# sloisel/LinearAlgebraMPI.jl

Hardware: AMD Instinct MI355X
Metric: SpMV GFLOP/s (2*nnz/t), 2-D 5-pt Poisson, fp64 (higher is better)
Workload: dtype f64

## Files before the change

include/hpcla_rocm.h:

```cpp
#ifndef HPCLA_ROCM_H
#define HPCLA_ROCM_H

#include <stdint.h>

#ifdef __cplusplus
extern "C" {
#endif

#define HPCLA_VERSION 100

#define HPCLA_OK 0
#define HPCLA_ERR_INVALID -1
#define HPCLA_ERR_HIP -2
#define HPCLA_ERR_RCCL -3
#define HPCLA_ERR_NO_DEVICE -4
#define HPCLA_ERR_UNSUPPORTED -5
#define HPCLA_ERR_ALLOC -6

#define HPCLA_LAYOUT_ROW 0
#define HPCLA_LAYOUT_COL 1

typedef struct hpcla_comm hpcla_comm_t;
typedef struct hpcla_halo_plan hpcla_halo_plan_t;

int hpcla_version(void);
const char *hpcla_last_error(void);
int hpcla_device_count(int *count);
int hpcla_set_device(int device);
int hpcla_device_info(int device, int *num_cus, char *arch_name_host, int arch_name_len);

int hpcla_spmv_csr_f64_i32(const int32_t *rowptr, const int32_t *colval, const double *nzval,
                           const double *x, double *y, int64_t nrows, int64_t nnz, int index_base,
                           void *stream);
int hpcla_spmv_csr_f64_i64(const int64_t *rowptr, const int64_t *colval, const double *nzval,
                           const double *x, double *y, int64_t nrows, int64_t nnz, int index_base,
                           void *stream);

int hpcla_spmv_split_f64_i32(const int32_t *rowptr, const int32_t *colval_split,
                             const double *nzval, const double *x_own, const double *x_ghost,
                             int64_t n_own, double *y, int64_t nrows, int64_t nnz, int index_base,
                             const int32_t *block_list, int64_t n_blocks, void *stream);
int hpcla_spmv_split_f64_i64(const int64_t *rowptr, const int64_t *colval_split,
                             const double *nzval, const double *x_own, const double *x_ghost,
                             int64_t n_own, double *y, int64_t nrows, int64_t nnz, int index_base,
                             const int32_t *block_list, int64_t n_blocks, void *stream);
int hpcla_spmv_rows_per_block(void);
int64_t hpcla_spmv_longrows_work_bytes(int64_t n_long);
int hpcla_spmv_longrows_f64_i32(const int32_t *rowptr, const int32_t *colval_split, const double *nzval,
                                const double *x_own, const double *x_ghost, int64_t n_own, double *y,
                                int64_t nrows, int64_t nnz, int index_base, const int64_t *long_rows,
                                int64_t n_long, int64_t long_min, double *work, void *stream);
int hpcla_spmv_longrows_f64_i64(const int64_t *rowptr, const int64_t *colval_split, const double *nzval,
                                const double *x_own, const double *x_ghost, int64_t n_own, double *y,
                                int64_t nrows, int64_t nnz, int index_base, const int64_t *long_rows,
                                int64_t n_long, int64_t long_min, double *work, void *stream);
int hpcla_spmm_rows_per_block(void);
int hpcla_spmm_block_order_hint(const void *rowptr, int group);
int hpcla_spmm_tune_block_order_f64_i32(const int32_t *rowptr, const int32_t *colval_split, const double *nzval,
                                        const double *B_own, int64_t ldb_own, const double *B_ghost, int64_t ldb_ghost,
                                        int64_t n_own, double *C, int64_t ldc, int64_t nrows, int64_t nnz, int k,
                                        int index_base, const int32_t *block_list, int64_t n_blocks, void *stream,
                                        int *chosen_group);
int hpcla_spmm_tune_block_order_f64_i64(const int64_t *rowptr, const int64_t *colval_split, const double *nzval,
                                        const double *B_own, int64_t ldb_own, const double *B_ghost, int64_t ldb_ghost,
                                        int64_t n_own, double *C, int64_t ldc, int64_t nrows, int64_t nnz, int k,
                                        int index_base, const int32_t *block_list, int64_t n_blocks, void *stream,
                                        int *chosen_group);

int hpcla_spmv_block_order_hint(const void *rowptr, int group);

int hpcla_spmv_tune_block_order_f64_i32(const int32_t *rowptr, const int32_t *colval_split, const double *nzval,
                                        const double *x_own, const double *x_ghost, int64_t n_own, double *y_scratch,
                                        int64_t nrows, int64_t nnz, int index_base, void *stream, int *chosen_group);
int hpcla_spmv_tune_block_order_f64_i64(const int64_t *rowptr, const int64_t *colval_split, const double *nzval,
                                        const double *x_own, const double *x_ghost, int64_t n_own, double *y_scratch,
                                        int64_t nrows, int64_t nnz, int index_base, void *stream, int *chosen_group);

int hpcla_remap_i32(const int32_t *in, const int32_t *map, int32_t *out, int64_t n, int index_base,
                    void *stream);
int hpcla_remap_i64(const int64_t *in, const int64_t *map, int64_t *out, int64_t n, int index_base,
                    void *stream);
int hpcla_remap_i64_to_i32(const int64_t *in, const int32_t *map, int32_t *out, int64_t n, int index_base,
                           void *stream);
int hpcla_narrow_i64_to_i32(const int64_t *in, int32_t *out, int64_t n, uint32_t *overflow_dev, void *stream);
int hpcla_classify_blocks_i32(const int32_t *rowptr, const int32_t *colval_split, int64_t nrows,
                              int index_base, int64_t n_own, int rows_per_block, int32_t *flags,
                              void *stream);
int hpcla_classify_blocks_i64(const int64_t *rowptr, const int64_t *colval_split, int64_t nrows,
                              int index_base, int64_t n_own, int rows_per_block, int32_t *flags,
                              void *stream);

int64_t hpcla_colspace_work_bytes(int64_t window);
int hpcla_digest_i32(const int32_t *a, int64_t n, uint64_t *out_host , void *stream);
int hpcla_digest_i64(const int64_t *a, int64_t n, uint64_t *out_host , void *stream);
int hpcla_compress_columns_i32(const int64_t *colidx_global, int64_t nnz, int64_t col_lo, int64_t window,
                               int32_t *colval_out, int index_base, int64_t *col_indices_out,
                               int64_t *ncols_compressed_host, void *work, void *stream);
int hpcla_compress_columns_i64(const int64_t *colidx_global, int64_t nnz, int64_t col_lo, int64_t window,
                               int64_t *colval_out, int index_base, int64_t *col_indices_out,
                               int64_t *ncols_compressed_host, void *work, void *stream);
int64_t hpcla_poisson2d_nnz(int64_t nx, int64_t ny, int64_t row_start, int64_t row_end);
int hpcla_gen_poisson2d(int64_t nx, int64_t ny, int64_t row_start, int64_t row_end, int64_t *rowptr_out,
                        int64_t *colidx_out, double *vals_out, void *stream);
int64_t hpcla_poisson3d_nnz(int64_t nx, int64_t ny, int64_t nz, int64_t row_start, int64_t row_end);
int hpcla_gen_poisson3d(int64_t nx, int64_t ny, int64_t nz, int64_t row_start, int64_t row_end,
                        int64_t *rowptr_out, int64_t *colidx_out, double *vals_out, void *stream);

int64_t hpcla_submatrix_work_bytes(int64_t nsel, int64_t width);
int64_t hpcla_submatrix_scan_chunk(void);
int hpcla_submatrix_structure_i32(const int32_t *rowptr, const int32_t *colval, int64_t nrows, int64_t nnz, int64_t r0,
                                  int64_t r1, int64_t j0, int64_t j1, int index_base, const int64_t *col_indices_src,
                                  int64_t col_shift, int64_t *src_start_out, int32_t *rowptr_out, int64_t *col_indices_out,
                                  int64_t *nnz_out_host, int64_t *ncols_out_host, void *work, void *stream);
int hpcla_submatrix_structure_i64(const int64_t *rowptr, const int64_t *colval, int64_t nrows, int64_t nnz, int64_t r0,
                                  int64_t r1, int64_t j0, int64_t j1, int index_base, const int64_t *col_indices_src,
                                  int64_t col_shift, int64_t *src_start_out, int64_t *rowptr_out, int64_t *col_indices_out,
                                  int64_t *nnz_out_host, int64_t *ncols_out_host, void *work, void *stream);
int hpcla_submatrix_fill_i32(int elem_bytes, const int32_t *colval, const void *nzval, int64_t nnz_src,
                             const int64_t *src_start, const int32_t *rowptr_out, int64_t nsel, int64_t nnz_out, int64_t j0,
                             int64_t j1, int index_base, const void *work, int32_t *colval_out, void *nzval_out, void *stream);
int hpcla_submatrix_fill_i64(int elem_bytes, const int64_t *colval, const void *nzval, int64_t nnz_src,
                             const int64_t *src_start, const int64_t *rowptr_out, int64_t nsel, int64_t nnz_out, int64_t j0,
                             int64_t j1, int index_base, const void *work, int64_t *colval_out, void *nzval_out, void *stream);
int hpcla_submatrix_values_i32(int elem_bytes, const void *nzval, int64_t nnz_src, const int64_t *src_start,
                               const int32_t *rowptr_out, int64_t nsel, int64_t nnz_out, int index_base, void *nzval_out,
                               void *stream);
int hpcla_submatrix_values_i64(int elem_bytes, const void *nzval, int64_t nnz_src, const int64_t *src_start,
                               const int64_t *rowptr_out, int64_t nsel, int64_t nnz_out, int index_base, void *nzval_out,
                               void *stream);
// ... 708 lines not shown
```

linearalgebrampi.jl_amd/_capi.py:

```python
from __future__ import annotations

import ctypes
import os

_HERE = os.path.dirname(os.path.abspath(__file__))
LIB_PATH = os.path.join(_HERE, "libhpcla_rocm.so")

OK = 0
LAYOUT_ROW = 0
LAYOUT_COL = 1
UNIQUE_ID_BYTES = 128
WINDOW_DESC_BYTES = 128
WINDOW_TABLE_ROWS = 4
COMM_NO_RCCL = 1
HALO_SINGLE_BUFFER = 1
BLOCK_PATTERNS_WEAK_HASH = 1


class HPCLAError(RuntimeError):
    def __init__(self, fn: str, status: int, text: str):
        super().__init__(f"{fn} failed with status {status}: {text}")
        self.status = status


_lib = None

_i32 = ctypes.c_int
_i64 = ctypes.c_int64
_u64 = ctypes.c_uint64
_f64 = ctypes.c_double
_f32 = ctypes.c_float
_vp = ctypes.c_void_p

_SIGNATURES = {
    "hpcla_version": [],
    "hpcla_last_error": [],
    "hpcla_device_count": [_vp],
    "hpcla_set_device": [_i32],
    "hpcla_device_info": [_i32, _vp, _vp, _i32],
    "hpcla_spmv_csr_f64_i32": [_vp, _vp, _vp, _vp, _vp, _i64, _i64, _i32, _vp],
    "hpcla_spmv_csr_f64_i64": [_vp, _vp, _vp, _vp, _vp, _i64, _i64, _i32, _vp],
    "hpcla_spmv_split_f64_i32": [_vp, _vp, _vp, _vp, _vp, _i64, _vp, _i64, _i64, _i32, _vp, _i64, _vp],
    "hpcla_spmv_split_f64_i64": [_vp, _vp, _vp, _vp, _vp, _i64, _vp, _i64, _i64, _i32, _vp, _i64, _vp],
    "hpcla_spmv_rows_per_block": [],
    "hpcla_spmv_longrows_work_bytes": [_i64],
    "hpcla_spmv_longrows_f64_i32": [_vp, _vp, _vp, _vp, _vp, _i64, _vp, _i64, _i64, _i32, _vp, _i64, _i64, _vp, _vp],
    "hpcla_spmv_longrows_f64_i64": [_vp, _vp, _vp, _vp, _vp, _i64, _vp, _i64, _i64, _i32, _vp, _i64, _i64, _vp, _vp],
    "hpcla_spmv_block_order_hint": [_vp, _i32],
    "hpcla_spmv_tune_block_order_f64_i32": [_vp, _vp, _vp, _vp, _vp, _i64, _vp, _i64, _i64, _i32, _vp, _vp],
    "hpcla_spmv_tune_block_order_f64_i64": [_vp, _vp, _vp, _vp, _vp, _i64, _vp, _i64, _i64, _i32, _vp, _vp],
    "hpcla_spmv_tune_block_order_cols16_f64_i32": [_vp, _vp, _vp, _vp, _vp, _i64, _i64, _i32, _i64, _i64, _vp, _vp],
    "hpcla_cols16_padded_len": [_i64],
    "hpcla_cols16_encode_i32": [_vp, _vp, _i64, _i64, _i64, _i32, _vp, _i64, _vp, _vp, _vp],
    "hpcla_spmv_cols16_f64_i32": [_vp, _vp, _vp, _vp, _vp, _i64, _i64, _i32, _vp, _i64, _vp],
    "hpcla_block_patterns_create_i32": [_vp, _vp, _vp, _i64, _i64, _i32, _vp, _i64, _i64, _i32, _vp],
    "hpcla_block_patterns_destroy": [_vp],
    "hpcla_block_patterns_info": [_vp, _vp, _vp, _vp, _vp],
    "hpcla_spmv_patterns_f64_i32": [_vp, _vp, _vp, _vp, _vp, _vp, _i64, _i64, _i32, _vp, _i64, _vp],
    "hpcla_spmv_tune_block_order_patterns_f64_i32": [_vp, _vp, _vp, _vp, _vp, _vp, _i64, _i64, _i32, _i64, _i64, _vp, _vp],
    "hpcla_spmm_rows_per_block": [],
    "hpcla_spmm_runs_desc_bytes": [_i64],
    "hpcla_spmm_runs_build_i32": [_vp, _vp, _i64, _i64, _i32, _i64, _vp, _vp, _vp],
    "hpcla_spmm_runs_build_i64": [_vp, _vp, _i64, _i64, _i32, _i64, _vp, _vp, _vp],
    "hpcla_spmm_banded_blocks_i32": [_vp, _vp, _i64, _i64, _i32, _i64, _i32, _vp, _vp],
    "hpcla_spmm_banded_blocks_i64": [_vp, _vp, _i64, _i64, _i32, _i64, _i32, _vp, _vp],
    "hpcla_spmm_runs_k16_f64_i32": [_vp, _vp, _vp, _vp, _vp, _i64, _vp, _i64, _i64, _i32, _vp, _vp, _i64, _vp],
    "hpcla_spmm_runs_k16_f64_i64": [_vp, _vp, _vp, _vp, _vp, _i64, _vp, _i64, _i64, _i32, _vp, _vp, _i64, _vp],
    "hpcla_spmm_runs_colmajor_k16_f64_i32": [_vp, _vp, _vp, _vp, _i64, _vp, _i64, _i64, _vp, _i64, _i64, _i64, _i32, _vp, _vp, _i64, _vp],
    "hpcla_spmm_runs_colmajor_k16_f64_i64": [_vp, _vp, _vp, _vp, _i64, _vp, _i64, _i64, _vp, _i64, _i64, _i64, _i32, _vp, _vp, _i64, _vp],
    "hpcla_spmm_runs_colmajor_tune_block_order_f64_i32": [_vp, _vp, _vp, _vp, _i64, _vp, _i64, _i64, _vp, _i64, _i64, _i64, _i32, _vp, _vp, _i64, _vp, _vp],
    "hpcla_spmm_runs_colmajor_tune_block_order_f64_i64": [_vp, _vp, _vp, _vp, _i64, _vp, _i64, _i64, _vp, _i64, _i64, _i64, _i32, _vp, _vp, _i64, _vp, _vp],
    "hpcla_spmm_block_order_hint": [_vp, _i32],
    "hpcla_spmm_tune_block_order_f64_i32": [_vp, _vp, _vp, _vp, _i64, _vp, _i64, _i64, _vp, _i64, _i64, _i64, _i32, _i32,
                                            _vp, _i64, _vp, _vp],
    "hpcla_spmm_tune_block_order_f64_i64": [_vp, _vp, _vp, _vp, _i64, _vp, _i64, _i64, _vp, _i64, _i64, _i64, _i32, _i32,
                                            _vp, _i64, _vp, _vp],
    "hpcla_remap_i32": [_vp, _vp, _vp, _i64, _i32, _vp],
    "hpcla_remap_i64": [_vp, _vp, _vp, _i64, _i32, _vp],
    "hpcla_remap_i64_to_i32": [_vp, _vp, _vp, _i64, _i32, _vp],
    "hpcla_narrow_i64_to_i32": [_vp, _vp, _i64, _vp, _vp],
    "hpcla_classify_blocks_i32": [_vp, _vp, _i64, _i32, _i64, _i32, _vp, _vp],
    "hpcla_classify_blocks_i64": [_vp, _vp, _i64, _i32, _i64, _i32, _vp, _vp],
    "hpcla_spmm_csr_f64_i32": [_vp, _vp, _vp, _vp, _i64, _i32, _vp, _i64, _i32, _i64, _i64, _i32, _i32, _vp],
    "hpcla_spmm_csr_f64_i64": [_vp, _vp, _vp, _vp, _i64, _i32, _vp, _i64, _i32, _i64, _i64, _i32, _i32, _vp],
    "hpcla_spmm_split_f64_i32": [_vp, _vp, _vp, _vp, _i64, _vp, _i64, _i64, _vp, _i64, _i64, _i64, _i32, _i32, _vp, _i64, _vp],
    "hpcla_spmm_split_f64_i64": [_vp, _vp, _vp, _vp, _i64, _vp, _i64, _i64, _vp, _i64, _i64, _i64, _i32, _i32, _vp, _i64, _vp],
    "hpcla_spmm_split_ccol_f64_i32": [_vp, _vp, _vp, _vp, _i64, _vp, _i64, _i64, _vp, _i64, _i64, _i64, _i32, _i32, _vp, _i64, _vp],
    "hpcla_spmm_split_ccol_f64_i64": [_vp, _vp, _vp, _vp, _i64, _vp, _i64, _i64, _vp, _i64, _i64, _i64, _i32, _i32, _vp, _i64, _vp],
    "hpcla_spmm_split_colmajor_f64_i32": [_vp, _vp, _vp, _vp, _i64, _vp, _i64, _i64, _vp, _i64, _i64, _i64, _i32, _i32, _vp, _i64, _vp],
    "hpcla_spmm_split_colmajor_f64_i64": [_vp, _vp, _vp, _vp, _i64, _vp, _i64, _i64, _vp, _i64, _i64, _i64, _i32, _i32, _vp, _i64, _vp],
    "hpcla_halo_begin_strided_f64": [_vp, _vp, _i64, _i64, _vp, _vp],
    "hpcla_spmm_panel_f64_i32": [_vp, _vp, _vp, _vp, _i64, _vp, _i64, _i64, _vp, _i64, _i64, _i64, _i32, _i32, _i32, _vp],
    "hpcla_spmm_panel_f64_i64": [_vp, _vp, _vp, _vp, _i64, _vp, _i64, _i64, _vp, _i64, _i64, _i64, _i32, _i32, _i32, _vp],
    "hpcla_transpose_f64": [_vp, _i64, _i32, _vp, _i64, _i32, _i64, _i64, _vp],
    "hpcla_gather_f64_i32": [_vp, _vp, _vp, _vp, _i64, _i32, _vp],
    "hpcla_gather_f64_i64": [_vp, _vp, _vp, _vp, _i64, _i32, _vp],
    "hpcla_comm_get_unique_id": [_vp],
    "hpcla_comm_init_rank": [_vp, _vp, _i32, _i32],
    "hpcla_comm_init_rank_ex": [_vp, _vp, _i32, _i32, _i32],
    "hpcla_comm_window_export": [_vp, _vp],
    "hpcla_comm_window_attach": [_vp, _vp],
# ... 259 lines not shown
    "hpcla_spmv_dot_work_bytes": _i64,
    "hpcla_colspace_work_bytes": _i64,
    "hpcla_submatrix_work_bytes": _i64,
    "hpcla_submatrix_scan_chunk": _i64,
    "hpcla_poisson2d_nnz": _i64,
    "hpcla_poisson3d_nnz": _i64,
    "hpcla_spgemm_bin_cap": _i64,
    "hpcla_gemv_t_work_bytes": _i64,
    "hpcla_gram_work_bytes": _i64,
    "hpcla_spmm_t_struct_work_bytes": _i64,
    "hpcla_spmm_runs_desc_bytes": _i64,
    "hpcla_spmv_longrows_work_bytes": _i64,
    "hpcla_cols16_padded_len": _i64,
    "hpcla_pcg_work_bytes": _i64,
    "hpcla_fsai_work_bytes": _i64,
    "hpcla_ilu_work_bytes": _i64,
    "hpcla_amg_work_bytes": _i64,
    "hpcla_amg_round_blocks": _i64,
    "hpcla_bicgstab_work_bytes": _i64,
    "hpcla_lsqr_work_bytes": _i64,
    "hpcla_minres_work_bytes": _i64,
    "hpcla_gmres_work_bytes": _i64,
    "hpcla_gmres_small_offset": _i64,
    "hpcla_eigsh_small_offset": _i64,
    "hpcla_svds_small_offset": _i64,
    "hpcla_lobpcg_chunk_rows": _i64,
    "hpcla_lobpcg_work_bytes": _i64,
    "hpcla_lobpcg_gen_work_bytes": _i64,
    "hpcla_qr_work_bytes": _i64,
}

EXPORTED_SYMBOLS = tuple(_SIGNATURES)


def load() -> ctypes.CDLL:
    global _lib
    if _lib is not None:
        return _lib
    if not os.path.exists(LIB_PATH):
        raise ImportError(
            f"{LIB_PATH} not found: build it with `python -c 'import __graft_entry__ as g; g.build()'` "
            "or `make -C linearalgebrampi.jl_amd/csrc` (hipcc --offload-arch=gfx950). "
            "There is no CPU fallback.")
    try:
        import torch
    except Exception:
        pass
    lib = ctypes.CDLL(LIB_PATH, mode=ctypes.RTLD_GLOBAL)
    for name, argtypes in _SIGNATURES.items():
        fn = getattr(lib, name)
        fn.argtypes = argtypes
        fn.restype = _RESTYPES.get(name, ctypes.c_int)
    _lib = lib
    return lib


def last_error() -> str:
    s = load().hpcla_last_error()
    return s.decode("utf-8", "replace") if s else ""


def check(fn_name: str, status: int) -> None:
    if status != OK:
        raise HPCLAError(fn_name, status, last_error())


def call(fn_name: str, *args) -> None:
    check(fn_name, getattr(load(), fn_name)(*args))
```

linearalgebrampi.jl_amd/csrc/spmv.hip:

```cpp
#include <stdlib.h>
#include <string.h>

#include <atomic>
#include <mutex>
#include <type_traits>
#include <unordered_map>

#include "common.h"
#include "halo_wait.h"
#include "patterns.h"

namespace hpcla {

constexpr int RPB = 256;
static_assert(RPB == PAT_RPB, "the pattern table is built for this kernel's row blocks");
constexpr int CHUNK = RPB * 8;
constexpr int UNROLL = CHUNK / RPB;

template <typename T, int N>
using vec = T __attribute__((ext_vector_type(N)));

struct Cols16 {};
struct Pat16 {};
template <typename P>
struct IndexPolicy {
    using row_t = P;
    using col_t = P;
    static constexpr int VEC = 4;
    static constexpr bool PATTERNS = false;
    static __device__ __forceinline__ int64_t decode(col_t c, int base, int64_t ) { return (int64_t)(P)(c - (P)base); }
    static __device__ __forceinline__ col_t fill(int base) { return (P)base; }
};
template <>
struct IndexPolicy<Cols16> {
    using row_t = int32_t;
    using col_t = int16_t;
    static constexpr int VEC = 8;
    static constexpr bool PATTERNS = false;
    static __device__ __forceinline__ int64_t decode(col_t d, int , int64_t r0) { return r0 + (int)d; }
    static __device__ __forceinline__ col_t fill(int ) { return 0; }
};
template <>
struct IndexPolicy<Pat16> : IndexPolicy<Cols16> {
    static constexpr bool PATTERNS = true;
};

template <bool SPLIT>
__device__ __forceinline__ double gather_x(const double *__restrict__ x_own,
                                           const double *__restrict__ x_ghost, int64_t n_own,
                                           int64_t col)
{
    if (SPLIT) {
        const double *p = col < n_own ? x_own + col : x_ghost + (col - n_own);
        return *p;
    }
    return x_own[col];
}

struct BlockSel {
    const int32_t *list;
    int64_t base;
    const int32_t *first_list;
    int64_t first_base;
    int64_t n_first;
    int64_t n_run;
    int32_t group_log2;
    int32_t nt_y;
};

constexpr int NUM_XCD_LOG2 = 3;
__device__ __forceinline__ int64_t xcd_group_index(int64_t b, int64_t n, int group_log2)
{
    const int64_t span = (int64_t)1 << (NUM_XCD_LOG2 + group_log2);
    if (b >= n - (n & (span - 1))) return b;
    const int64_t xcd = b & ((1 << NUM_XCD_LOG2) - 1), q = b >> NUM_XCD_LOG2;
    return ((((q >> group_log2) << NUM_XCD_LOG2) + xcd) << group_log2) + (q & (((int64_t)1 << group_log2) - 1));
}

template <bool WAIT>
__device__ __forceinline__ int64_t select_block(const BlockSel &bs, bool &wait, int lead)
{
    const int64_t b = (int64_t)blockIdx.x - lead;
    wait = false;
    if (WAIT) {
        if (b < bs.n_first) {
            if (bs.first_list) return (int64_t)bs.first_list[b];
            return bs.first_base + (bs.group_log2 > 0 ? xcd_group_index(b, bs.n_run, bs.group_log2) : b);
        }
        wait = true;
        return bs.list ? (int64_t)bs.list[b - bs.n_first] : bs.base + (b - bs.n_first);
    }
    if (bs.list) return (int64_t)bs.list[b];
    return bs.base + (bs.group_log2 > 0 ? xcd_group_index(b, bs.n_run, bs.group_log2) : b);
}

__device__ __forceinline__ void block_dot_epilogue(double *s_scratch, double *__restrict__ dot_partial,
                                                   int64_t blk, double v)
{
#pragma unroll
    for (int off = 32; off > 0; off >>= 1) v += __shfl_down(v, off, 64);
    const int lane = threadIdx.x & 63, w = threadIdx.x >> 6;
    if (lane == 0) s_scratch[w] = v;
    __syncthreads();
    if (threadIdx.x == 0) dot_partial[blk] = ((s_scratch[0] + s_scratch[1]) + s_scratch[2]) + s_scratch[3];
}

constexpr int RG_CHW = 464;
constexpr int RG_UR = 8;

template <typename I, bool SPLIT, bool WAIT, bool LONGR = false>
__global__ __launch_bounds__(RPB) void spmv_rowgather_kernel(
    const typename IndexPolicy<I>::row_t *__restrict__ rowptr, const typename IndexPolicy<I>::col_t *__restrict__ colval,
    const double *__restrict__ nzval, const double *__restrict__ x_own, const double *x_ghost, int64_t n_own,
    double *__restrict__ y, int64_t nrows, int64_t nnz, int base,
    BlockSel bs, double *__restrict__ dot_partial, HaloWait hw, PushArgs push, int64_t long_min = 0, PatArgs pat = PatArgs{nullptr, nullptr})
{
    using IP = IndexPolicy<I>;
    using R = typename IP::row_t;
    using C = typename IP::col_t;
    constexpr int V = IP::VEC;
    constexpr int NV = (RG_CHW / V + 63) / 64;
    static_assert(!LONGR || !WAIT, "the long-row form is a plain launch");
    static_assert(V * sizeof(C) == 16 || sizeof(C) == 8, "one 16-byte column load per staged vector (Int64: two)");
    static_assert(RG_CHW % V == 0 && RG_CHW >= 64 * 7 + V - 1, "a pass holds a 7-entry stencil's wave behind any aligned start");
    __shared__ __attribute__((aligned(16))) C s_col_all[(RPB / 64) * RG_CHW];
    __shared__ __attribute__((aligned(16))) double s_val_all[(RPB / 64) * RG_CHW];
    __shared__ double s_red[RPB / 64];

    if constexpr (WAIT) {
        if ((int)blockIdx.x < push.n_blocks) {
            halo_push_block<R, RPB>(push, (int)blockIdx.x);
            return;
        }
    }
    const int tid = threadIdx.x;
    bool wait_ghosts;
    const int64_t blk = select_block<WAIT>(bs, wait_ghosts, WAIT ? push.n_blocks : 0);
    uint32_t waited = 0;
    if (WAIT && wait_ghosts) {
        waited = halo_wait_block(hw, hw.first_wait_reader + (uint32_t)(blockIdx.x - push.n_blocks - bs.n_first));
        x_ghost = hw.ghost0 + (int64_t)(waited & ~HALO_WAIT_TIMED_OUT) * hw.buf_stride;
    }
    const int64_t r0 = blk * RPB;
    const int nr = (int)((nrows - r0) < RPB ? (nrows - r0) : RPB);
    if (WAIT && (waited & HALO_WAIT_TIMED_OUT)) {
        if ((int)threadIdx.x < nr) y[r0 + threadIdx.x] = halo_poison();
// ... 86 lines not shown
            {
                R blo = rlo, bhi = rhi;
                if constexpr (IP::PATTERNS)
                    if (!streamed) {
                        blo = roff + (R)((uint32_t)rlo & 0xffffu);
                        bhi = roff + (R)((uint32_t)rlo >> 16);
                    }
                const int64_t lo64 = lane < nrw ? (int64_t)blo - base - pa - c : 0;
                const int64_t hi64 = lane < nrw ? (int64_t)bhi - base - pa - c : 0;
                const int lo = lo64 < 0 ? 0 : (lo64 > n ? n : (int)lo64);
                const int hi = hi64 < 0 ? 0 : (hi64 > n ? n : (int)hi64);
                const uint64_t whole = __ballot(lane < nrw && lo == 0 && hi == n && !(LONGR && is_long));
                if (whole) {
#pragma unroll 4
                    for (int e = lane; e < n; e += 64)
                        s_val[e] = s_val[e] * gather_x<SPLIT>(x_own, x_ghost, n_own, IP::decode(s_col[e], base, r0));
                    __builtin_amdgcn_fence(__ATOMIC_RELEASE, "wavefront");
                    __builtin_amdgcn_wave_barrier();
                    if (lane == __ffsll((unsigned long long)whole) - 1) {
                        int j = 0;
#pragma unroll 1
                        for (; j + 4 <= n; j += 4) {
                            const double p0 = s_val[j], p1 = s_val[j + 1], p2 = s_val[j + 2], p3 = s_val[j + 3];
                            acc += p0; acc += p1; acc += p2; acc += p3;
                        }
#pragma unroll 1
                        for (; j < n; ++j) acc += s_val[j];
                    }
                    __builtin_amdgcn_fence(__ATOMIC_ACQUIRE, "wavefront");
                    __builtin_amdgcn_wave_barrier();
                    continue;
                }
                int j = lo;
                int e = hi;
                if (LONGR && is_long) e = j;
                for (; j < e; j += RG_UR) {
                    int64_t cc[RG_UR];
                    double vv[RG_UR], xx[RG_UR];
#pragma unroll
                    for (int u = 0; u < RG_UR; ++u) {
                        cc[u] = 0; vv[u] = 0.0;
                        if (j + u < e) { cc[u] = IP::decode(s_col[j + u], base, r0); vv[u] = s_val[j + u]; }
                    }
#pragma unroll
                    for (int u = 0; u < RG_UR; ++u) { xx[u] = 0.0; if (j + u < e) xx[u] = gather_x<SPLIT>(x_own, x_ghost, n_own, cc[u]); }
#pragma unroll
                    for (int u = 0; u < RG_UR; ++u) if (j + u < e) acc += vv[u] * xx[u];
                }
            }
            __builtin_amdgcn_fence(__ATOMIC_ACQUIRE, "wavefront");
            __builtin_amdgcn_wave_barrier();
        }
        if (lane < nrw && !(LONGR && is_long)) {
            if (bs.nt_y) __builtin_nontemporal_store(acc, y + rw + lane);
            else y[rw + lane] = acc;
        } else if (LONGR && lane < nrw) {
            y[rw + lane] = __builtin_nan("");
        }
    }
    if (dot_partial) block_dot_epilogue(s_red, dot_partial, blk, lane < nrw ? acc * x_row : 0.0);
}

constexpr int LR_CHUNKS = 1024;
constexpr int64_t LR_MIN_CHUNK = 4096;

template <typename I, bool SPLIT>
__global__ __launch_bounds__(256) void spmv_longrow_partial_kernel(
    const I *__restrict__ rowptr, const I *__restrict__ colval, const double *__restrict__ nzval,
    const double *__restrict__ x_own, const double *x_ghost, int64_t n_own, int base,
    const int64_t *__restrict__ long_rows, double *__restrict__ partial)
{
    __shared__ double s_w[4];
    const int64_t r = long_rows[blockIdx.y];
    const int64_t p0 = (int64_t)rowptr[r] - base, p1 = (int64_t)rowptr[r + 1] - base, len = p1 - p0;
    int64_t chunk = (len + LR_CHUNKS - 1) / LR_CHUNKS;
    if (chunk < LR_MIN_CHUNK) chunk = LR_MIN_CHUNK;
    const int64_t s = p0 + (int64_t)blockIdx.x * chunk;
    const int64_t e = s + chunk < p1 ? s + chunk : p1;
    double a0 = 0.0, a1 = 0.0, a2 = 0.0, a3 = 0.0;
    int64_t i = s + threadIdx.x;
    for (; i + 768 < e; i += 1024) {
        const int64_t c0 = (int64_t)(I)(colval[i] - (I)base), c1 = (int64_t)(I)(colval[i + 256] - (I)base),
                      c2 = (int64_t)(I)(colval[i + 512] - (I)base), c3 = (int64_t)(I)(colval[i + 768] - (I)base);
        const double v0 = nzval[i], v1 = nzval[i + 256], v2 = nzval[i + 512], v3 = nzval[i + 768];
        a0 += v0 * gather_x<SPLIT>(x_own, x_ghost, n_own, c0);
        a1 += v1 * gather_x<SPLIT>(x_own, x_ghost, n_own, c1);
        a2 += v2 * gather_x<SPLIT>(x_own, x_ghost, n_own, c2);
        a3 += v3 * gather_x<SPLIT>(x_own, x_ghost, n_own, c3);
    }
    for (; i < e; i += 256) a0 += nzval[i] * gather_x<SPLIT>(x_own, x_ghost, n_own, (int64_t)(I)(colval[i] - (I)base));
    double v = (a0 + a1) + (a2 + a3);
#pragma unroll
    for (int off = 32; off > 0; off >>= 1) v += __shfl_down(v, off, 64);
    if ((threadIdx.x & 63) == 0) s_w[threadIdx.x >> 6] = v;
    __syncthreads();
    if (threadIdx.x == 0) partial[(int64_t)blockIdx.y * LR_CHUNKS + blockIdx.x] = ((s_w[0] + s_w[1]) + s_w[2]) + s_w[3];
}

__global__ __launch_bounds__(256) void spmv_longrow_final_kernel(const int64_t *__restrict__ long_rows,
                                                                 const double *__restrict__ partial, double *__restrict__ y)
{
    __shared__ double s_w[4];
    static_assert(LR_CHUNKS == 1024, "four pieces per thread");
    const double *p = partial + (int64_t)blockIdx.x * LR_CHUNKS + threadIdx.x * 4;
    double v = ((p[0] + p[1]) + p[2]) + p[3];
#pragma unroll
    for (int off = 32; off > 0; off >>= 1) v += __shfl_down(v, off, 64);
// ... 114 lines not shown
    if (threadIdx.x == 0) flags[blockIdx.x] = any ? 1 : 0;
}

template <typename I>
__global__ __launch_bounds__(256) void gather_kernel(const double *__restrict__ x,
                                                     const I *__restrict__ src,
                                                     const I *__restrict__ dst,
                                                     double *__restrict__ out, int64_t n, int base)
{
    int64_t i = (int64_t)blockIdx.x * blockDim.x + threadIdx.x;
    const int64_t stride = (int64_t)gridDim.x * blockDim.x;
    for (; i < n; i += stride) {
        const int64_t d = dst ? (int64_t)dst[i] - base : i;
        out[d] = x[(int64_t)src[i] - base];
    }
}

static inline uint32_t stream_grid(int64_t n, int threads)
{
    int64_t g = (n + threads - 1) / threads;
    if (g < 1) g = 1;
    if (g > 256 * 16) g = 256 * 16;
    return (uint32_t)g;
}

static std::mutex g_order_mu;
static std::unordered_map<const void *, int> g_order;
static std::atomic<int> g_order_count{0};

static int block_order_of(const void *rowptr)
{
    static const int forced = [] {
        const char *e = getenv("HPCLA_SPMV_XCD_GROUP");
        int g = e ? atoi(e) : 0, l = 0;
        while (g > 1) { g >>= 1; ++l; }
        return l > 10 ? 10 : l;
    }();
    if (forced) return forced;
    if (g_order_count.load(std::memory_order_relaxed) == 0) return 0;
    std::lock_guard<std::mutex> lock(g_order_mu);
    auto it = g_order.find(rowptr);
    return it == g_order.end() ? 0 : it->second;
}

static int spmv_nt_y(bool )
{
    static const int on = [] {
        const char *e = getenv("HPCLA_SPMV_NT_Y");
        return e ? (atoi(e) ? 1 : 0) : 1;
    }();
    return on;
}

template <typename I>
static int spmv_launch(const typename IndexPolicy<I>::row_t *rowptr, const typename IndexPolicy<I>::col_t *colval,
                       const double *nzval, const double *x_own,
                       const double *x_ghost, int64_t n_own, bool split, double *y, int64_t nrows,
                       int64_t nnz, int index_base, const int32_t *block_list, int64_t n_blocks,
                       void *stream, double *dot_partial = nullptr, int64_t block_base = -1, const PatArgs *pat = nullptr)
{
    if (nrows < 0 || nnz < 0) return set_error(HPCLA_ERR_INVALID, "spmv: negative size");
    if (index_base != 0 && index_base != 1)
        return set_error(HPCLA_ERR_INVALID, "spmv: index_base must be 0 or 1");
    if (nrows == 0) return HPCLA_OK;
    if (!rowptr || !y) return set_error(HPCLA_ERR_INVALID, "spmv: null rowptr/y");
    if (nnz > 0 && (!colval || !nzval || !x_own))
        return set_error(HPCLA_ERR_INVALID, "spmv: null colval/nzval/x with nnz > 0");
    const int64_t all_blocks = (nrows + RPB - 1) / RPB;
    int64_t launch_blocks = all_blocks;
    if (block_list) {
        if (n_blocks < 0 || n_blocks > all_blocks)
            return set_error(HPCLA_ERR_INVALID, "spmv: n_blocks out of range");
        launch_blocks = n_blocks;
        block_base = 0;
    } else if (block_base >= 0) {
        if (n_blocks < 0 || block_base + n_blocks > all_blocks)
            return set_error(HPCLA_ERR_INVALID, "spmv: block range out of bounds");
        launch_blocks = n_blocks;
    } else {
        block_base = 0;
    }
    if (launch_blocks == 0) return HPCLA_OK;
    if (launch_blocks > 0x7fffffffLL) return set_error(HPCLA_ERR_INVALID, "spmv: too many blocks");
    dim3 grid((uint32_t)launch_blocks), block(RPB);
    hipStream_t s = as_stream(stream);
    if (split && !x_ghost) split = false;
    using IP = IndexPolicy<I>;
    const bool aligned = (reinterpret_cast<uintptr_t>(colval) % (IP::VEC * sizeof(typename IP::col_t)) == 0) &&
                         (reinterpret_cast<uintptr_t>(nzval) % 32 == 0);
    const BlockSel bs{block_list, block_base, nullptr, 0, 0, launch_blocks, block_list ? 0 : block_order_of(rowptr),
                      spmv_nt_y(dot_partial != nullptr)};
    HaloWait nowait;
    memset(&nowait, 0, sizeof(nowait));
    PushArgs nopush;
    memset(&nopush, 0, sizeof(nopush));
    if constexpr (std::is_same<I, Cols16>::value) {
        if (!aligned) return set_error(HPCLA_ERR_INVALID, "spmv: 16-bit columns need a 16-byte aligned copy and 32-byte aligned nzval");
        if (pat)
            spmv_rowgather_kernel<Pat16, false, false><<<grid, block, 0, s>>>(
                rowptr, colval, nzval, x_own, nullptr, 0, y, nrows, nnz, index_base, bs, dot_partial, nowait, nopush, 0, *pat);
        else
            spmv_rowgather_kernel<Cols16, false, false><<<grid, block, 0, s>>>(
                rowptr, colval, nzval, x_own, nullptr, 0, y, nrows, nnz, index_base, bs, dot_partial, nowait, nopush);
    } else if (aligned) {
        if (split)
            spmv_rowgather_kernel<I, true, false><<<grid, block, 0, s>>>(
                rowptr, colval, nzval, x_own, x_ghost, n_own, y, nrows, nnz, index_base, bs, dot_partial, nowait, nopush);
        else
            spmv_rowgather_kernel<I, false, false><<<grid, block, 0, s>>>(
                rowptr, colval, nzval, x_own, nullptr, 0, y, nrows, nnz, index_base, bs, dot_partial, nowait, nopush);
    } else {
        if (split)
            spmv_rowblock_kernel<I, true, false><<<grid, block, 0, s>>>(
                rowptr, colval, nzval, x_own, x_ghost, n_own, y, nrows, index_base, bs, dot_partial, nowait, nopush);
        else
            spmv_rowblock_kernel<I, false, false><<<grid, block, 0, s>>>(
                rowptr, colval, nzval, x_own, nullptr, 0, y, nrows, index_base, bs, dot_partial, nowait, nopush);
    }
    HPCLA_CHECK_LAUNCH();
    return HPCLA_OK;
}

template <typename I>
static int spmv_launch_fused(const I *rowptr, const I *colval, const double *nzval, const double *x_own,
                             const double *x_ghost, int64_t n_own, double *y, int64_t nrows, int64_t nnz,
                             int index_base, const int32_t *interior_list, int64_t interior_base,
                             int64_t n_interior, const int32_t *boundary_list, int64_t n_boundary,
                             const HaloWait &hw, const PushArgs &pa, void *stream, double *dot_partial)
{
    if (nrows < 0 || nnz < 0) return set_error(HPCLA_ERR_INVALID, "spmv: negative size");
    if (index_base != 0 && index_base != 1)
        return set_error(HPCLA_ERR_INVALID, "spmv: index_base must be 0 or 1");
    if (nrows > 0 && (!rowptr || !y)) return set_error(HPCLA_ERR_INVALID, "spmv: null rowptr/y");
    if (nnz > 0 && (!colval || !nzval || !x_own))
        return set_error(HPCLA_ERR_INVALID, "spmv: null colval/nzval/x with nnz > 0");
    const int64_t all_blocks = (nrows + RPB - 1) / RPB;
    if (n_interior < 0 || n_boundary < 0 || n_interior + n_boundary > all_blocks)
        return set_error(HPCLA_ERR_INVALID, "spmv: block counts out of range");
    if (n_boundary > 0 && !boundary_list) return set_error(HPCLA_ERR_INVALID, "spmv: null boundary list");
    if (n_boundary > 0 && !x_ghost) return set_error(HPCLA_ERR_INVALID, "spmv: boundary blocks without a ghost segment");
    if (!interior_list && n_interior > 0 && (interior_base < 0 || interior_base + n_interior > all_blocks))
        return set_error(HPCLA_ERR_INVALID, "spmv: interior run out of bounds");
    const int64_t launch_blocks = pa.n_blocks + n_interior + n_boundary;
    if (launch_blocks == 0) return HPCLA_OK;
    if (launch_blocks > 0x7fffffffLL) return set_error(HPCLA_ERR_INVALID, "spmv: too many blocks");
    dim3 grid((uint32_t)launch_blocks), block(RPB);
    hipStream_t s = as_stream(stream);
    const bool aligned = (reinterpret_cast<uintptr_t>(colval) % (4 * sizeof(I)) == 0) &&
                         (reinterpret_cast<uintptr_t>(nzval) % 32 == 0);
    const BlockSel bs{boundary_list, 0, interior_list, interior_base, n_interior, n_interior,
// ... 59 lines not shown
    for (int64_t j = p0 + threadIdx.x; j < p1; j += 256) {
        const int64_t c = (int64_t)colval[j] - base;
        const int64_t d = c - r0;
        if (c < 0 || c >= n_own || d < -32768 || d > 32767) bad = 1;
        dcol[j] = (int16_t)d;
    }
    if (__syncthreads_or(bad) && threadIdx.x == 0) atomicOr(flags, 1);
}

int64_t cols16_padded_len(int64_t nnz) { return ((nnz + 7) / 8) * 8 + 8; }

int encode_cols16_i32(const int32_t *rowptr, const int32_t *colval, int64_t nrows, int index_base, int64_t n_own,
                      const int32_t *block_list, int64_t n_blocks, int16_t *dcol, int *flag_dev, void *stream)
{
    if (n_blocks <= 0) return HPCLA_OK;
    encode_cols_kernel<<<(uint32_t)n_blocks, 256, 0, as_stream(stream)>>>(rowptr, colval, nrows, index_base, n_own, block_list,
                                                                         dcol, flag_dev);
    HPCLA_CHECK_LAUNCH();
    return HPCLA_OK;
}

int patterns_args(const hpcla_block_patterns *p, int64_t nrows, int64_t nnz, int index_base, PatArgs *out);

bool cols16_usable(const int16_t *cols16, const double *nzval)
{
    return cols16 && reinterpret_cast<uintptr_t>(cols16) % 16 == 0 && reinterpret_cast<uintptr_t>(nzval) % 32 == 0;
}

int spmv_cols16_i32(const int32_t *rowptr, const int16_t *cols16, const double *nzval, const double *x, double *y,
                    int64_t nrows, int64_t nnz, int index_base, const int32_t *bl, int64_t nb, void *stream,
                    double *dot_partial, int64_t block_base, const hpcla_block_patterns *patterns)
{
    PatArgs pa;
    if (patterns)
        if (const int rc = patterns_args(patterns, nrows, nnz, index_base, &pa)) return rc;
    return spmv_launch<Cols16>(rowptr, cols16, nzval, x, nullptr, 0, false, y, nrows, nnz, index_base, bl, nb, stream,
                               dot_partial, block_base, patterns ? &pa : nullptr);
}

}

using namespace hpcla;

HPCLA_API int hpcla_spmv_rows_per_block(void) { return RPB; }

static void set_block_order(const void *rowptr, int group_log2)
{
    std::lock_guard<std::mutex> lock(g_order_mu);
    if (group_log2 <= 0) g_order.erase(rowptr);
    else g_order[rowptr] = group_log2;
    g_order_count.store((int)g_order.size(), std::memory_order_relaxed);
}

template <typename I>
static int tune_block_order(const typename IndexPolicy<I>::row_t *rowptr, const typename IndexPolicy<I>::col_t *colval_split,
                            const double *nzval, const double *x_own,
                            const double *x_ghost, int64_t n_own, double *y_scratch, int64_t nrows, int64_t nnz,
                            int index_base, void *stream, int *chosen_group, int64_t run_base = -1, int64_t run_blocks = 0,
                            const PatArgs *pat = nullptr)
{
    if (chosen_group) *chosen_group = 1;
    if (nrows < 0 || nnz < 0 || !rowptr) return set_error(HPCLA_ERR_INVALID, "spmv_tune_block_order: bad arguments");
    set_block_order(rowptr, 0);
    const int64_t n_blocks = (nrows + RPB - 1) / RPB;
    if (n_blocks < 4096 || nnz == 0) return HPCLA_OK;
    if (run_base >= 0 && (run_blocks <= 0 || run_base + run_blocks > n_blocks))
        return run_blocks == 0 ? HPCLA_OK : set_error(HPCLA_ERR_INVALID, "spmv_tune_block_order: block run out of bounds");
    if (!y_scratch) return set_error(HPCLA_ERR_INVALID, "spmv_tune_block_order: null scratch vector");
    constexpr int NC = 4, ROUNDS = 4, REPS = 4;
    const int cand[NC] = {0, 3, 5, 6};
    float ms[NC][ROUNDS];
    hipEvent_t e0, e1;
    HPCLA_CHECK_HIP(hipEventCreate(&e0));
    HPCLA_CHECK_HIP(hipEventCreate(&e1));
    hipStream_t s = as_stream(stream);
    int rc = HPCLA_OK;
    for (int r = 0; r < ROUNDS && rc == HPCLA_OK; ++r)
        for (int c = 0; c < NC && rc == HPCLA_OK; ++c) {
            set_block_order(rowptr, cand[c]);
            if (hipEventRecord(e0, s) != hipSuccess) { rc = set_error(HPCLA_ERR_HIP, "spmv_tune_block_order: event"); break; }
            for (int i = 0; i < REPS && rc == HPCLA_OK; ++i)
                rc = spmv_launch<I>(rowptr, colval_split, nzval, x_own, x_ghost, n_own, true, y_scratch, nrows, nnz,
                                    index_base, nullptr, run_base >= 0 ? run_blocks : 0, stream, nullptr, run_base, pat);
            if (rc != HPCLA_OK) break;
            if (hipEventRecord(e1, s) != hipSuccess || hipEventSynchronize(e1) != hipSuccess ||
                hipEventElapsedTime(&ms[c][r], e0, e1) != hipSuccess)
                rc = set_error(HPCLA_ERR_HIP, "spmv_tune_block_order: timing");
        }
    (void)hipEventDestroy(e0);
    (void)hipEventDestroy(e1);
    set_block_order(rowptr, 0);
    if (rc != HPCLA_OK) return rc;
    float best_t[NC];
    for (int c = 0; c < NC; ++c) {
        float a = ms[c][1], b = ms[c][2], d = ms[c][3];
        best_t[c] = a > b ? (b > d ? b : (a > d ? d : a)) : (a > d ? a : (b > d ? d : b));
    }
    int best = 0;
    for (int c = 1; c < NC; ++c)
        if (best_t[c] < best_t[best]) best = c;
    if (best != 0 && best_t[best] > 0.99f * best_t[0]) best = 0;
    set_block_order(rowptr, cand[best]);
    if (chosen_group) *chosen_group = 1 << cand[best];
    return HPCLA_OK;
}

HPCLA_API int hpcla_spmv_tune_block_order_f64_i32(const int32_t *rowptr, const int32_t *colval_split, const double *nzval,
                                                  const double *x_own, const double *x_ghost, int64_t n_own,
                                                  double *y_scratch, int64_t nrows, int64_t nnz, int index_base,
                                                  void *stream, int *chosen_group)
{
    return tune_block_order<int32_t>(rowptr, colval_split, nzval, x_own, x_ghost, n_own, y_scratch, nrows, nnz, index_base,
                                     stream, chosen_group);
}

HPCLA_API int hpcla_spmv_tune_block_order_f64_i64(const int64_t *rowptr, const int64_t *colval_split, const double *nzval,
                                                  const double *x_own, const double *x_ghost, int64_t n_own,
                                                  double *y_scratch, int64_t nrows, int64_t nnz, int index_base,
                                                  void *stream, int *chosen_group)
{
    return tune_block_order<int64_t>(rowptr, colval_split, nzval, x_own, x_ghost, n_own, y_scratch, nrows, nnz, index_base,
                                     stream, chosen_group);
}

HPCLA_API int hpcla_spmv_tune_block_order_cols16_f64_i32(const int32_t *rowptr, const int16_t *cols16, const double *nzval,
                                                         const double *x_own, double *y_scratch, int64_t nrows, int64_t nnz,
                                                         int index_base, int64_t block_base, int64_t n_blocks, void *stream,
                                                         int *chosen_group)
{
    if (!cols16_usable(cols16, nzval))
        return set_error(HPCLA_ERR_INVALID, "spmv_tune_block_order_cols16: null or misaligned column copy / nzval");
    return tune_block_order<Cols16>(rowptr, cols16, nzval, x_own, nullptr, 0, y_scratch, nrows, nnz, index_base, stream,
                                    chosen_group, block_base, n_blocks);
}

HPCLA_API int hpcla_spmv_tune_block_order_patterns_f64_i32(const int32_t *rowptr, const int16_t *cols16,
                                                           const hpcla_block_patterns_t *patterns, const double *nzval,
                                                           const double *x_own, double *y_scratch, int64_t nrows, int64_t nnz,
                                                           int index_base, int64_t block_base, int64_t n_blocks, void *stream,
                                                           int *chosen_group)
{
    if (!cols16_usable(cols16, nzval))
        return set_error(HPCLA_ERR_INVALID, "spmv_tune_block_order_patterns: null or misaligned column copy / nzval");
    PatArgs pa;
    if (patterns)
        if (const int rc = patterns_args(patterns, nrows, nnz, index_base, &pa)) return rc;
    return tune_block_order<Cols16>(rowptr, cols16, nzval, x_own, nullptr, 0, y_scratch, nrows, nnz, index_base, stream,
                                    chosen_group, block_base, n_blocks, patterns ? &pa : nullptr);
}

HPCLA_API int64_t hpcla_cols16_padded_len(int64_t nnz) { return cols16_padded_len(nnz > 0 ? nnz : 0); }

HPCLA_API int hpcla_cols16_encode_i32(const int32_t *rowptr, const int32_t *colval_split, int64_t nrows, int64_t nnz,
                                      int64_t n_own, int index_base, const int32_t *block_list, int64_t n_blocks,
                                      int16_t *cols16, int *ineligible_dev, void *stream)
{
// ... 241 lines not shown
```

Measured before the change: 1000.

## Alternate SpMV block sweep direction across repeated calls and harden block-order tuner

Repeated SpMV launches on the same matrix and range now alternate between forward and reversed block order, while keeping each XCD's block interleave intact. The aim is that data touched at the end of one sweep, still resident in L2 or Infinity Cache, is read first by the next sweep. This saves part of the HBM traffic for matrices slightly larger than cache. The block-order tuner now runs a warm-up round, uses more rounds and an even number of reps so both directions are timed equally, and picks a candidate only if it wins every round on the median ratio. The cost is per-thread state that tracks the last call, plus an env switch to turn the behaviour off.

```diff
diff --git a/include/hpcla_rocm.h b/include/hpcla_rocm.h
--- a/include/hpcla_rocm.h
+++ b/include/hpcla_rocm.h
@@ -75,6 +75,11 @@
 int hpcla_spmv_tune_block_order_f64_i64(const int64_t *rowptr, const int64_t *colval_split, const double *nzval,
                                         const double *x_own, const double *x_ghost, int64_t n_own, double *y_scratch,
                                         int64_t nrows, int64_t nnz, int index_base, void *stream, int *chosen_group);
+
+int hpcla_block_order_decide(const float *ms, int n_cand, int n_rounds, int *chosen_index);
+
+int hpcla_set_spmv_sweep(int mode);
+int hpcla_spmv_last_sweep(int *reversed);
 
 int hpcla_remap_i32(const int32_t *in, const int32_t *map, int32_t *out, int64_t n, int index_base,
                     void *stream);
diff --git a/linearalgebrampi.jl_amd/_capi.py b/linearalgebrampi.jl_amd/_capi.py
--- a/linearalgebrampi.jl_amd/_capi.py
+++ b/linearalgebrampi.jl_amd/_capi.py
@@ -47,6 +47,9 @@
     "hpcla_spmv_longrows_f64_i32": [_vp, _vp, _vp, _vp, _vp, _i64, _vp, _i64, _i64, _i32, _vp, _i64, _i64, _vp, _vp],
     "hpcla_spmv_longrows_f64_i64": [_vp, _vp, _vp, _vp, _vp, _i64, _vp, _i64, _i64, _i32, _vp, _i64, _i64, _vp, _vp],
     "hpcla_spmv_block_order_hint": [_vp, _i32],
+    "hpcla_block_order_decide": [_vp, _i32, _i32, _vp],
+    "hpcla_set_spmv_sweep": [_i32],
+    "hpcla_spmv_last_sweep": [_vp],
     "hpcla_spmv_tune_block_order_f64_i32": [_vp, _vp, _vp, _vp, _vp, _i64, _vp, _i64, _i64, _i32, _vp, _vp],
     "hpcla_spmv_tune_block_order_f64_i64": [_vp, _vp, _vp, _vp, _vp, _i64, _vp, _i64, _i64, _i32, _vp, _vp],
     "hpcla_spmv_tune_block_order_cols16_f64_i32": [_vp, _vp, _vp, _vp, _vp, _i64, _i64, _i32, _i64, _i64, _vp, _vp],
@@ -412,7 +415,13 @@
         fn.argtypes = argtypes
         fn.restype = _RESTYPES.get(name, ctypes.c_int)
     _lib = lib
+    apply_spmv_sweep_env()
     return lib
+
+
+def apply_spmv_sweep_env() -> None:
+    want = os.environ.get("HPCLA_SPMV_SWEEP", "alternate").strip().lower()
+    call("hpcla_set_spmv_sweep", 0 if want.startswith("f") else -1)
 
 
 def last_error() -> str:
diff --git a/linearalgebrampi.jl_amd/csrc/spmv.hip b/linearalgebrampi.jl_amd/csrc/spmv.hip
--- a/linearalgebrampi.jl_amd/csrc/spmv.hip
+++ b/linearalgebrampi.jl_amd/csrc/spmv.hip
@@ -67,6 +67,8 @@
     int32_t group_log2;
     int32_t nt_y;
 };
+constexpr int32_t BS_NT_Y = 1;
+constexpr int32_t BS_REVERSED = 2;
 
 constexpr int NUM_XCD_LOG2 = 3;
 __device__ __forceinline__ int64_t xcd_group_index(int64_t b, int64_t n, int group_log2)
@@ -75,6 +77,12 @@
     if (b >= n - (n & (span - 1))) return b;
     const int64_t xcd = b & ((1 << NUM_XCD_LOG2) - 1), q = b >> NUM_XCD_LOG2;
     return ((((q >> group_log2) << NUM_XCD_LOG2) + xcd) << group_log2) + (q & (((int64_t)1 << group_log2) - 1));
+}
+
+__device__ __forceinline__ int64_t reversed_index(int64_t b, int64_t n)
+{
+    const int64_t xcd = b & ((1 << NUM_XCD_LOG2) - 1), q = b >> NUM_XCD_LOG2;
+    return ((((n - xcd + ((1 << NUM_XCD_LOG2) - 1)) >> NUM_XCD_LOG2) - 1 - q) << NUM_XCD_LOG2) + xcd;
 }
 
 template <bool WAIT>
@@ -91,7 +99,8 @@
         return bs.list ? (int64_t)bs.list[b - bs.n_first] : bs.base + (b - bs.n_first);
     }
     if (bs.list) return (int64_t)bs.list[b];
-    return bs.base + (bs.group_log2 > 0 ? xcd_group_index(b, bs.n_run, bs.group_log2) : b);
+    const int64_t c = (bs.nt_y & BS_REVERSED) ? reversed_index(b, bs.n_run) : b;
+    return bs.base + (bs.group_log2 > 0 ? xcd_group_index(c, bs.n_run, bs.group_log2) : c);
 }
 
 __device__ __forceinline__ void block_dot_epilogue(double *s_scratch, double *__restrict__ dot_partial,
@@ -284,7 +293,7 @@
             __builtin_amdgcn_wave_barrier();
         }
         if (lane < nrw && !(LONGR && is_long)) {
-            if (bs.nt_y) __builtin_nontemporal_store(acc, y + rw + lane);
+            if (bs.nt_y & BS_NT_Y) __builtin_nontemporal_store(acc, y + rw + lane);
             else y[rw + lane] = acc;
         } else if (LONGR && lane < nrw) {
             y[rw + lane] = __builtin_nan("");
@@ -505,6 +514,26 @@
     return on;
 }
 
+enum { SWEEP_FORWARD = 0, SWEEP_ALTERNATE = 1 };
+static std::atomic<int> g_sweep_mode{SWEEP_ALTERNATE};
+static int sweep_mode() { return g_sweep_mode.load(std::memory_order_relaxed); }
+
+struct SweepRecord {
+    const void *rowptr, *nzval;
+    int64_t nrows, base, len;
+    int reversed;
+};
+static thread_local SweepRecord t_sweep = {nullptr, nullptr, 0, 0, 0, 0};
+
+static int next_sweep(const void *rowptr, const void *nzval, int64_t nrows, int64_t base, int64_t len)
+{
+    SweepRecord &t = t_sweep;
+    const bool again = t.rowptr == rowptr && t.nzval == nzval && t.nrows == nrows && t.base == base && t.len == len;
+    const int reversed = (again && sweep_mode() == SWEEP_ALTERNATE) ? !t.reversed : 0;
+    t = SweepRecord{rowptr, nzval, nrows, base, len, reversed};
+    return reversed;
+}
+
 template <typename I>
 static int spmv_launch(const typename IndexPolicy<I>::row_t *rowptr, const typename IndexPolicy<I>::col_t *colval,
                        const double *nzval, const double *x_own,
@@ -541,14 +570,16 @@
     using IP = IndexPolicy<I>;
     const bool aligned = (reinterpret_cast<uintptr_t>(colval) % (IP::VEC * sizeof(typename IP::col_t)) == 0) &&
                          (reinterpret_cast<uintptr_t>(nzval) % 32 == 0);
+    if (std::is_same<I, Cols16>::value && !aligned)
+        return set_error(HPCLA_ERR_INVALID, "spmv: 16-bit columns need a 16-byte aligned copy and 32-byte aligned nzval");
+    const int reversed = block_list ? 0 : next_sweep(rowptr, nzval, nrows, block_base, launch_blocks);
     const BlockSel bs{block_list, block_base, nullptr, 0, 0, launch_blocks, block_list ? 0 : block_order_of(rowptr),
-                      spmv_nt_y(dot_partial != nullptr)};
+                      spmv_nt_y(dot_partial != nullptr) | (reversed ? BS_REVERSED : 0)};
     HaloWait nowait;
     memset(&nowait, 0, sizeof(nowait));
     PushArgs nopush;
     memset(&nopush, 0, sizeof(nopush));
     if constexpr (std::is_same<I, Cols16>::value) {
-        if (!aligned) return set_error(HPCLA_ERR_INVALID, "spmv: 16-bit columns need a 16-byte aligned copy and 32-byte aligned nzval");
         if (pat)
             spmv_rowgather_kernel<Pat16, false, false><<<grid, block, 0, s>>>(
                 rowptr, colval, nzval, x_own, nullptr, 0, y, nrows, nnz, index_base, bs, dot_partial, nowait, nopush, 0, *pat);
@@ -714,6 +745,41 @@
     g_order_count.store((int)g_order.size(), std::memory_order_relaxed);
 }
 
+constexpr int DECIDE_MAX_ROUNDS = 64;
+static int block_order_decide(const float *ms, int n_cand, int n_rounds, int *chosen_index)
+{
+    if (!ms || !chosen_index || n_cand < 1 || n_rounds < 1 || n_rounds > DECIDE_MAX_ROUNDS)
+        return set_error(HPCLA_ERR_INVALID, "block_order_decide: null table, or n_cand < 1, or n_rounds outside 1 ... 64");
+    for (int i = 0; i < n_cand * n_rounds; ++i)
+        if (!(ms[i] > 0.0f) || ms[i] > 3.0e38f) return set_error(HPCLA_ERR_INVALID, "block_order_decide: times must be positive and finite");
+    int best = 0;
+    double best_ratio = 0.99;
+    bool have = false;
+    for (int c = 1; c < n_cand; ++c) {
+        double ratio[DECIDE_MAX_ROUNDS];
+        bool every_round = true;
+        for (int r = 0; r < n_rounds; ++r) {
+            ratio[r] = (double)ms[c * n_rounds + r] / (double)ms[r];
+            every_round = every_round && ratio[r] < 1.0;
+        }
+        if (!every_round) continue;
+        for (int i = 1; i < n_rounds; ++i)
+            for (int j = i; j > 0 && ratio[j] < ratio[j - 1]; --j) {
+                const double t = ratio[j];
+                ratio[j] = ratio[j - 1];
+                ratio[j - 1] = t;
+            }
+        const double med = (n_rounds & 1) ? ratio[n_rounds / 2] : 0.5 * (ratio[n_rounds / 2 - 1] + ratio[n_rounds / 2]);
+        if (have ? med < best_ratio : med <= best_ratio) {
+            best = c;
+            best_ratio = med;
+            have = true;
+        }
+    }
+    *chosen_index = best;
+    return HPCLA_OK;
+}
+
 template <typename I>
 static int tune_block_order(const typename IndexPolicy<I>::row_t *rowptr, const typename IndexPolicy<I>::col_t *colval_split,
                             const double *nzval, const double *x_own,
@@ -729,41 +795,54 @@
     if (run_base >= 0 && (run_blocks <= 0 || run_base + run_blocks > n_blocks))
         return run_blocks == 0 ? HPCLA_OK : set_error(HPCLA_ERR_INVALID, "spmv_tune_block_order: block run out of bounds");
     if (!y_scratch) return set_error(HPCLA_ERR_INVALID, "spmv_tune_block_order: null scratch vector");
-    constexpr int NC = 4, ROUNDS = 4, REPS = 4;
+    constexpr int NC = 4, ROUNDS = 5, TUNE_REPS = 8, WARM_REPS = 2;
+    static_assert(TUNE_REPS % 2 == 0 && WARM_REPS % 2 == 0, "every window sees both sweep directions equally");
     const int cand[NC] = {0, 3, 5, 6};
-    float ms[NC][ROUNDS];
+    float ms[NC * ROUNDS], warm;
     hipEvent_t e0, e1;
     HPCLA_CHECK_HIP(hipEventCreate(&e0));
     HPCLA_CHECK_HIP(hipEventCreate(&e1));
     hipStream_t s = as_stream(stream);
     int rc = HPCLA_OK;
-    for (int r = 0; r < ROUNDS && rc == HPCLA_OK; ++r)
+    for (int r = -1; r < ROUNDS && rc == HPCLA_OK; ++r)
         for (int c = 0; c < NC && rc == HPCLA_OK; ++c) {
             set_block_order(rowptr, cand[c]);
             if (hipEventRecord(e0, s) != hipSuccess) { rc = set_error(HPCLA_ERR_HIP, "spmv_tune_block_order: event"); break; }
-            for (int i = 0; i < REPS && rc == HPCLA_OK; ++i)
+            for (int i = 0; i < (r < 0 ? WARM_REPS : TUNE_REPS) && rc == HPCLA_OK; ++i)
                 rc = spmv_launch<I>(rowptr, colval_split, nzval, x_own, x_ghost, n_own, true, y_scratch, nrows, nnz,
                                     index_base, nullptr, run_base >= 0 ? run_blocks : 0, stream, nullptr, run_base, pat);
             if (rc != HPCLA_OK) break;
             if (hipEventRecord(e1, s) != hipSuccess || hipEventSynchronize(e1) != hipSuccess ||
-                hipEventElapsedTime(&ms[c][r], e0, e1) != hipSuccess)
+                hipEventElapsedTime(r < 0 ? &warm : &ms[c * ROUNDS + r], e0, e1) != hipSuccess)
                 rc = set_error(HPCLA_ERR_HIP, "spmv_tune_block_order: timing");
         }
     (void)hipEventDestroy(e0);
     (void)hipEventDestroy(e1);
     set_block_order(rowptr, 0);
     if (rc != HPCLA_OK) return rc;
-    float best_t[NC];
-    for (int c = 0; c < NC; ++c) {
-        float a = ms[c][1], b = ms[c][2], d = ms[c][3];
-        best_t[c] = a > b ? (b > d ? b : (a > d ? d : a)) : (a > d ? a : (b > d ? d : b));
-    }
     int best = 0;
-    for (int c = 1; c < NC; ++c)
-        if (best_t[c] < best_t[best]) best = c;
-    if (best != 0 && best_t[best] > 0.99f * best_t[0]) best = 0;
+    if ((rc = block_order_decide(ms, NC, ROUNDS, &best)) != HPCLA_OK) return rc;
     set_block_order(rowptr, cand[best]);
     if (chosen_group) *chosen_group = 1 << cand[best];
+    return HPCLA_OK;
+}
+
+HPCLA_API int hpcla_block_order_decide(const float *ms, int n_cand, int n_rounds, int *chosen_index)
+{
+    return block_order_decide(ms, n_cand, n_rounds, chosen_index);
+}
+
+HPCLA_API int hpcla_set_spmv_sweep(int mode)
+{
+    if (mode < -1 || mode > 1) return set_error(HPCLA_ERR_INVALID, "set_spmv_sweep: mode must be -1 (the default), 0 (forward) or 1 (alternate)");
+    g_sweep_mode.store(mode < 0 ? (int)SWEEP_ALTERNATE : mode, std::memory_order_relaxed);
+    return HPCLA_OK;
+}
+
+HPCLA_API int hpcla_spmv_last_sweep(int *reversed)
+{
+    if (!reversed) return set_error(HPCLA_ERR_INVALID, "spmv_last_sweep: null output");
+    *reversed = t_sweep.reversed;
     return HPCLA_OK;
 }
 
```

Result: faster. 1059 (median of 6 runs) (+5.9%).
